# zhouxuguang/GNXRayTracer

Hardware: AMD Instinct MI355X
Metric: Mrays/sec + wall-clock to 1024spp, dragon Cornell 1920×1080 (higher is better)
Workload: dtype f32; 1 GPU; cfg3: Cornell + synthetic 100000-tri mesh (stand-in for absent dragon.3d), Glass+Metal, PathIntegrator maxDepth 8 rr 1 spatial, Halton(1024), 1920x1080; passes_in_flight=4, sub_passes=56, spp_rendered=1024, gather=n/a, world_size=1, backend=none, devices_visible=1

## Files before the change

gnxraytracer_amd/__init__.py:

```python
import collections
import ctypes as C
import os

import numpy as np

from . import _abi
from ._abi import (Camera, Hit, Light, LiSample, Material, Medium, Ray, RenderParams, SceneDesc, Stats, Texture)

_HERE = os.path.dirname(os.path.abspath(__file__))
LIB_PATH = os.environ.get("GNXR_LIB", os.path.join(_HERE, "libgnxr.so"))


class GnxrError(RuntimeError):
    pass


_lib = None
_device = 0


def lib():
    global _lib
    if _lib is None:
        if not os.path.exists(LIB_PATH):
# ... 265 lines not shown
            if d.lights[i].type == _abi.LIGHT_INFINITE:
                self._env_light = Light()
                C.memmove(C.byref(self._env_light), C.byref(d.lights[i]), C.sizeof(Light))
                break
        self._textures = []
        for i in range(int(d.n_textures)):
            t = Texture()
            C.memmove(C.byref(t), C.byref(d.textures[i]), C.sizeof(Texture))
            t.texel_offset = 0
            self._textures.append(t)
        _check(lib().gnxr_scene_create(C.byref(d), C.byref(self._h)))

    def close(self):
        if getattr(self, "_h", None) and _lib is not None:
            _lib.gnxr_scene_destroy(self._h)
            self._h = None

    __del__ = close

    def info(self):
        n, dmax, nv = C.c_int32(), C.c_int32(), C.c_int32()
        _check(lib().gnxr_scene_info(self._h, C.byref(n), C.byref(dmax), C.byref(nv)))
        return {"bvh_nodes": n.value, "bvh_max_depth": dmax.value, "light_voxels": nv.value}

    def update_vertices(self, xyz, first_vertex=0, stream=None, move_lights=False):
        if isinstance(xyz, np.ndarray):
            if xyz.dtype != np.float32 or xyz.ndim != 2 or xyz.shape[1] != 3:
                raise ValueError(f"update_vertices: expected a float32 array of shape (n, 3), got {xyz.dtype} {xyz.shape}")
            xyz = np.ascontiguousarray(xyz)
            ptr = xyz.ctypes.data
        elif type(xyz).__module__.split(".")[0] == "torch":
            import torch
            if not (isinstance(xyz, torch.Tensor) and xyz.is_cuda and xyz.device.index == self.device and xyz.dtype == torch.float32 and
                    xyz.dim() == 2 and xyz.shape[1] == 3 and xyz.is_contiguous()):
                raise ValueError(f"update_vertices: expected a contiguous float32 (n, 3) tensor on cuda:{self.device}, got "
                                 f"{getattr(xyz, 'dtype', None)} {tuple(getattr(xyz, 'shape', ()))} on {getattr(xyz, 'device', None)}")
            ptr = xyz.data_ptr()
            if stream is None:
                stream = torch.cuda.current_stream(xyz.device)
        else:
            raise ValueError(f"update_vertices: expected a numpy array or a torch tensor, got {type(xyz).__name__}")
        stream = _stream_handle("update_vertices", stream)
        if move_lights:
            _check(lib().gnxr_scene_update_vertices_ex(self._h, int(first_vertex), int(xyz.shape[0]), C.c_void_p(ptr or None), _abi.UPDATE_MOVE_LIGHTS,
                                                       C.c_void_p(stream or None)))
        else:
# ... 1041 lines not shown
```

gnxraytracer_amd/_abi.py:

```python
import ctypes as C

GNXR_ABI_VERSION = 5

OK, ERR_INVALID, ERR_NO_DEVICE, ERR_OOM, ERR_UNSUPPORTED, ERR_IO, ERR_RUNTIME = 0, -1, -2, -3, -4, -5, -6
MAT_NONE, MAT_MATTE, MAT_MIRROR, MAT_GLASS, MAT_METAL, MAT_PLASTIC, MAT_DISNEY = range(7)
LIGHT_AREA_TRI, LIGHT_INFINITE, LIGHT_SKYBOX, LIGHT_POINT, LIGHT_SPOT, LIGHT_DISTANT = 1, 2, 3, 4, 5, 6
INTEGRATOR_PATH, INTEGRATOR_VOLPATH, INTEGRATOR_WHITTED, INTEGRATOR_DIRECT = 0, 1, 2, 3
DIRECT_SAMPLE_ALL, DIRECT_SAMPLE_ONE = 0, 1
LIGHTS_SPATIAL, LIGHTS_UNIFORM, LIGHTS_POWER = 0, 1, 2
MEDIUM_HOMOGENEOUS, MEDIUM_GRID = 1, 2
DMEDIUM_BYTES = 128
DLIGHT_BYTES = 112
DTEXTURE_BYTES = 112
UPDATE_MOVE_LIGHTS = 1

f32, i32, u8, i64, u32, u64 = C.c_float, C.c_int32, C.c_uint8, C.c_int64, C.c_uint32, C.c_uint64


class Material(C.Structure):
    _fields_ = [
        ("type", i32), ("has_bump", i32), ("remap_roughness", i32), ("disney_thin", i32),
        ("kd", f32 * 3), ("ks", f32 * 3), ("kr", f32 * 3), ("kt", f32 * 3), ("eta", f32 * 3), ("k", f32 * 3),
        ("sigma", f32), ("urough", f32), ("vrough", f32),
        ("disney_metallic", f32), ("disney_spec_trans", f32), ("disney_spec_tint", f32), ("disney_sheen", f32),
# ... 140 lines not shown
    "gnxr_scene_create": (C.c_int, [P(SceneDesc), P(VP)]),
    "gnxr_scene_destroy": (None, [VP]),
    "gnxr_scene_info": (C.c_int, [VP, P(i32), P(i32), P(i32)]),
    "gnxr_scene_update_vertices": (C.c_int, [VP, i32, i32, VP, VP]),
    "gnxr_scene_update_vertices_ex": (C.c_int, [VP, i32, i32, VP, u32, VP]),
    "gnxr_scene_update_lights": (C.c_int, [VP, i32, i32, P(Light)]),
    "gnxr_scene_set_lights": (C.c_int, [VP, P(Light), i32, VP]),
    "gnxr_scene_light_tables": (C.c_int, [VP, i32, VP, i64, P(i64)]),
    "gnxr_scene_rebuild_bvh": (C.c_int, [VP, VP]),
    "gnxr_scene_set_geometry": (C.c_int, [VP, P(Geometry), VP]),
    "gnxr_scene_update_environment": (C.c_int, [VP, P(Light), VP, i32, i32, VP]),
    "gnxr_scene_env_tables": (C.c_int, [VP, i32, VP, i64, P(i64)]),
    "gnxr_scene_update_media": (C.c_int, [VP, i32, i32, P(Medium), VP, VP]),
    "gnxr_scene_media_tables": (C.c_int, [VP, i32, i32, VP, i64, P(i64)]),
    "gnxr_scene_update_textures": (C.c_int, [VP, i32, i32, P(Texture), VP, VP]),
    "gnxr_scene_texture_tables": (C.c_int, [VP, i32, i32, VP, i64, P(i64)]),
    "gnxr_scene_update_materials": (C.c_int, [VP, i32, i32, P(Material)]),
    "gnxr_scene_set_triangle_materials": (C.c_int, [VP, i32, i32, VP, VP]),
    "gnxr_scene_triangle_materials": (C.c_int, [VP, P(i32), P(C.c_uint8), C.c_int64]),
    "gnxr_scene_set_camera": (C.c_int, [VP, P(Camera), i32]),
    "gnxr_render": (C.c_int, [VP, P(RenderParams), P(f32), P(Stats)]),
    "gnxr_render_device": (C.c_int, [VP, P(RenderParams), VP, VP, P(Stats)]),
    "gnxr_render_reserve": (C.c_int, [VP, P(RenderParams)]),
    "gnxr_trace_closest": (C.c_int, [VP, P(Ray), i64, P(Hit)]),
    "gnxr_trace_any": (C.c_int, [VP, P(Ray), i64, P(u8)]),
    "gnxr_trace_closest_device": (C.c_int, [VP, VP, i64, VP, VP]),
    "gnxr_trace_any_device": (C.c_int, [VP, VP, i64, VP, VP]),
    "gnxr_li_device": (C.c_int, [VP, P(RenderParams), VP, VP, i64, VP, VP, P(Stats)]),
    "gnxr_render_views_device": (C.c_int, [VP, P(RenderParams), P(Camera), P(i32), i32, VP, VP, P(Stats)]),
    "gnxr_render_aov_device": (C.c_int, [VP, P(RenderParams), P(Camera), P(i32), i32, P(AovBuffers), VP, P(Stats)]),
    "gnxr_render_adaptive_device": (C.c_int, [VP, P(RenderParams), P(AdaptiveParams), VP, VP, VP, P(Stats), P(AdaptiveInfo)]),
    "gnxr_denoise_device": (C.c_int, [P(DenoiseParams), P(DenoiseBuffers), VP, VP]),
    "gnxr_film_filter_table": (C.c_int, [P(FilmFilter), P(f32)]),
    "gnxr_film_add_device": (C.c_int, [P(FilmFilter), i32, i32, i32, i32, VP, VP, VP, VP]),
    "gnxr_film_resolve_device": (C.c_int, [i32, i32, i32, VP, VP, VP]),
    "gnxr_render_filtered_device": (C.c_int, [VP, P(RenderParams), P(FilmFilter), P(Camera), P(i32), i32, VP, VP, u32, VP, P(Stats)]),
    "gnxr_material_albedo": (C.c_int, [P(Material), P(f32)]),
    "gnxr_camera_rays_device": (C.c_int, [P(Camera), i32, i32, i32, VP, VP, VP, i64, VP, VP, VP]),
    "gnxr_bsdf_device": (C.c_int, [VP, VP, VP, VP, VP, i64, i32, VP, VP]),
    "gnxr_light_sample_device": (C.c_int, [VP, VP, i64, i32, VP, VP]),
    "gnxr_light_le_device": (C.c_int, [VP, i32, VP, i64, VP, VP]),
    "gnxr_sample_halton": (C.c_int, [i32, i32, P(i32), P(i32), P(i64), P(i32), i64, P(f32)]),
    "gnxr_camera_rays": (C.c_int, [P(Camera), i32, i32, P(i32), P(i32), P(i64), i64, P(f32), P(f32)]),
    "gnxr_framebuffer_update": (C.c_int, [P(f32), P(f32), i32, i32, i32, P(u8)]),
    "gnxr_framebuffer_save_png": (C.c_int, [C.c_char_p, P(u8), i32, i32]),
    "gnxr_light_grid_table": (C.c_int, [VP, i32, i32, P(f32), i64, P(i64)]),
# ... 52 lines not shown
```

gnxraytracer_amd/csrc/api.hip:

```cpp
#include <hip/hip_runtime.h>

#include <chrono>
#include <cstdio>
#include <cstdlib>
#include <memory>
#include <mutex>
#include <string>
#include <thread>
#include <vector>

#include "host_scene.h"
#include "kernels.hip.h"
#include "trace4_kernel.hip.h"
#include "hlbvh_build.hip.h"
#include "refit_kernel.hip.h"
#include "material_kernel.hip.h"
#include "rebuild_kernel.hip.h"
#include "geometry_kernel.hip.h"
#include "lights_kernel.hip.h"
#include "env_build_kernel.hip.h"
#include "media_kernel.hip.h"
#include "texture_build_kernel.hip.h"
#include "li_kernel.hip.h"
#include "views_kernel.hip.h"
// ... 142 lines not shown
    if (rc) return rc;
    gnxr_scene *s = new (std::nothrow) gnxr_scene(g_device);
    if (!s) return GNXR_ERR_OOM;
    if (!compile_scene(desc, &s->cs, device_hlbvh_build)) { delete s; return GNXR_ERR_INVALID; }
    for (size_t i = 1; i < g_devices.size(); ++i) s->replicas.push_back(std::make_unique<gnxr_scene>(g_devices[i], s->host));
    if ((rc = s->each_copy(upload_scene)) != GNXR_OK) { delete s; return rc; }
    const CompiledScene &cs = s->cs;
    if (getenv("GNXR_VERBOSE"))
        fprintf(stderr, "[gnxr] scene: %zu tris, %zu nodes (depth %d), %zu 4-wide nodes (stack %d), wide=%d, %zu device(s)\n", cs.tris.size(), cs.nodes.size(), cs.bvh_max_depth,
                cs.nodes4.size(), cs.stack4_need, (int)s->wide_ok, s->n_copies());
    *out = s;
    return GNXR_OK;
}
void gnxr_scene_destroy(gnxr_scene *s) { delete s; }

int gnxr_scene_info(const gnxr_scene *s, int32_t *n_nodes, int32_t *max_depth, int32_t *n_vox) {
    if (!s) return GNXR_ERR_INVALID;
    if (n_nodes) *n_nodes = (int32_t)s->cs.nodes.size();
    if (max_depth) *max_depth = s->cs.bvh_max_depth;
    if (n_vox) *n_vox = s->grid_strategy >= 0 ? s->grid.nvox[0] * s->grid.nvox[1] * s->grid.nvox[2] : 0;
    return GNXR_OK;
}

int gnxr_render_device(gnxr_scene *s, const gnxr_render_params *pin, void *d_rgba_out, void *hip_stream, gnxr_stats *stats) {
    return render_sharded(s, pin, d_rgba_out, hip_stream, stats);
}

int gnxr_render_reserve(gnxr_scene *s, const gnxr_render_params *pin) {
    if (!s || !pin) { set_error("null argument"); return GNXR_ERR_INVALID; }
    int dummy = 0;
    return render_sharded(s, pin, &dummy, nullptr, nullptr, true);
}

int gnxr_render(gnxr_scene *s, const gnxr_render_params *p, float *rgba_out, gnxr_stats *stats) {
    if (!s || !p || !rgba_out) { set_error("null argument"); return GNXR_ERR_INVALID; }
    if (p->width <= 0 || p->height <= 0) { set_error("invalid image size"); return GNXR_ERR_INVALID; }
    size_t npx = (size_t)p->width * p->height;
    std::lock_guard<std::recursive_mutex> lock(s->render_mutex);
    if (int brc = s->bind()) return brc;
    const bool grew = !(s->out.p && npx <= s->out.n);
    int rc = s->out.alloc(npx);
    if (rc) return rc;
    HIP_TRY(hipMemset(s->out.p, 0, npx * sizeof(float4)));
    rc = render_sharded(s, p, s->out.p, nullptr, stats);
    if (rc) { if (grew) s->out.release(); return rc; }
    int sc = p->shard_count > 0 ? p->shard_count : 1, sr = p->shard_rows > 0 ? p->shard_rows : 1;
// ... 254 lines not shown
```

gnxraytracer_amd/csrc/api_common.hip.h:

```cpp
#pragma once

namespace { int hip_status(hipError_t e); }
#define HIP_TRY(expr)                                                                                   \
    do {                                                                                                \
        hipError_t e_ = (expr);                                                                         \
        if (e_ != hipSuccess) {                                                                         \
            set_error("%s failed: %s (%s:%d)", #expr, hipGetErrorString(e_), __FILE__, __LINE__);       \
            return hip_status(e_);                                                                      \
        }                                                                                               \
    } while (0)

namespace {

int hip_status(hipError_t e) {
    if (e == hipErrorOutOfMemory) return GNXR_ERR_OOM;
    if (e == hipErrorNoDevice || e == hipErrorInvalidDevice || e == hipErrorInsufficientDriver || e == hipErrorNotInitialized) return GNXR_ERR_NO_DEVICE;
    return GNXR_ERR_RUNTIME;
}

int g_device = -1;
std::vector<int> g_devices;
std::vector<char> g_peer_ok;
int g_num_cus = 256;
int g_profiling = 0;
// ... 27 lines not shown
#define GX_ONCE(type, expr) do { static const type v = (expr); return v; } while (0)
    static int trace_blocks_per_cu() { const int v = env_int("GNXR_TRACE_BLOCKS_PER_CU", 0); return v >= 1 && v <= 8 ? v : 0; }
    static int grid_blocks_per_cu() { const int v = env_int("GNXR_GRID_BLOCKS_PER_CU", 0); return v >= 1 && v <= 4096 ? v : 0; }
    static int trace_lds_levels() { GX_ONCE(int, env_set("GNXR_TRACE_LDS_LEVELS") ? std::max(2, env_int("GNXR_TRACE_LDS_LEVELS", 0)) : 64); }
    static int trace_chunk() { GX_ONCE(int, env_set("GNXR_TRACE_CHUNK") ? std::max(64, env_int("GNXR_TRACE_CHUNK", 0) / 64 * 64) : kTraceChunk); }
    static bool leaf_box_table() { GX_ONCE(bool, env_set("GNXR_LEAF_BOX_TABLE")); }
    static int regions() { GX_ONCE(int, env_int("GNXR_REGIONS", 0)); }
    static bool pipeline() { GX_ONCE(bool, env_int("GNXR_PIPELINE", 1) != 0); }
    static int pipe_cut() { GX_ONCE(int, env_int("GNXR_PIPE_CUT", -1)); }
    static int loop_lag() { GX_ONCE(int, env_int("GNXR_LOOP_LAG", -1)); }
    static int shade_blocks_per_cu() { GX_ONCE(int, env_set("GNXR_SHADE_BLOCKS_PER_CU") ? std::max(1, env_int("GNXR_SHADE_BLOCKS_PER_CU", 0)) : 32); }
    static int shade_lds_dims() { GX_ONCE(int, env_set("GNXR_SHADE_LDS_DIMS") ? std::max(0, std::min(128, env_int("GNXR_SHADE_LDS_DIMS", 0))) : 64); }
    static bool shade_lds_tables() { GX_ONCE(bool, env_int("GNXR_SHADE_LDS_TABLES", 1) != 0); }
    static int shade_streams() { GX_ONCE(int, env_int("GNXR_SHADE_STREAMS", -1)); }
    static bool vol_pack() { GX_ONCE(bool, env_int("GNXR_VOL_PACK", 1) != 0); }
#undef GX_ONCE
    static int volmedia_step_cap() { return env_set("GNXR_VOLMEDIA_STEP_CAP") ? std::max(0, env_int("GNXR_VOLMEDIA_STEP_CAP", 0)) : 64; }
    static bool no_escape_queue() { return env_set("GNXR_NO_ESCAPE_QUEUE"); }
    static bool no_material_queues() { return env_set("GNXR_NO_MATERIAL_QUEUES"); }
    static bool no_narrow_shade() { return env_set("GNXR_NO_NARROW_SHADE"); }
    static bool no_mis_defer() { return env_set("GNXR_NO_MIS_DEFER"); }
    static int mis_defer_step() { const int v = env_int("GNXR_MIS_DEFER_STEP", 2); return v == 1 ? 1 : 2; }
    static int mis_defer_drain_at() { return std::max(1, std::min(64, env_int("GNXR_MIS_DEFER_DRAIN_AT", 64))); }
    static bool host_light_grid() { return env_set("GNXR_HOST_LIGHT_GRID"); }
    static bool binary_bvh() { return env_set("GNXR_BINARY_BVH"); }
};

int ensure_device() {
    if (g_device >= 0) { HIP_TRY(hipSetDevice(g_device)); return GNXR_OK; }
    int n = 0;
    hipError_t e = hipGetDeviceCount(&n);
    if (e != hipSuccess || n <= 0) {
        set_error("no HIP device available (%s); libgnxr has no CPU fallback", e != hipSuccess ? hipGetErrorString(e) : "0 devices");
        return GNXR_ERR_NO_DEVICE;
    }
    int dev = 0;
    HIP_TRY(hipGetDevice(&dev));
    hipDeviceProp_t prop;
    HIP_TRY(hipGetDeviceProperties(&prop, dev));
    g_num_cus = prop.multiProcessorCount > 0 ? prop.multiProcessorCount : 256;
    g_device = dev;
    if (const int v = Knobs::trace_blocks_per_cu()) g_trace_blocks_per_cu = v;
    if (const int v = Knobs::grid_blocks_per_cu()) g_grid_bpc = v;
    return GNXR_OK;
}

// ... 32 lines not shown
```

gnxraytracer_amd/csrc/api_render.hip.h:

```cpp
#pragma once

struct TraceLaunch {
    int entries;
    int lds_entries;
    bool spill_needed;
    size_t lds;
    int n_top;
    int blocks;
};
static TraceLaunch trace_launch(const gnxr_scene *s, bool wide, bool spheres, long long total) {
    TraceLaunch t;
    t.entries = wide ? s->cs.stack4_need + 1 : s->cs.bvh_max_depth + 2;
    const int per_cu = g_trace_blocks_per_cu;
    const size_t fixed_b = wide ? (size_t)(kRayRecDwords + (spheres ? 1 : 0)) * kRqStride * sizeof(int) + (size_t)kTopCache * 128 + kOrderTableBytes : 0;
    t.lds_entries = std::min(std::min(t.entries, Knobs::trace_lds_levels()), std::max(2, (int)(((160 * 1024) / per_cu - 1024 - fixed_b) / (kBlock * sizeof(int)))));
    t.spill_needed = t.entries > t.lds_entries;
    t.lds = (size_t)t.lds_entries * kBlock * sizeof(int) + fixed_b;
    t.n_top = (int)std::min<size_t>(kTopCache, s->cs.root4 >= 0 ? s->cs.nodes4.size() : 0);
    t.blocks = (int)std::min<long long>((long long)g_num_cus * per_cu, (total + kBlock - 1) / kBlock);
    return t;
}

static int count_local_rows(const gnxr_render_params *p) {
    int rows = 0;
// ... 526 lines not shown

#define GX_CHECK_LAUNCHES(where)                                                                                    \
    do {                                                                                                            \
        const hipError_t le_ = hipGetLastError();                                                                   \
        if (le_ != hipSuccess) { set_error("HIP runtime error in " where ": %s", hipGetErrorString(le_)); return hip_status(le_); } \
    } while (0)

static int run_path_loop(RenderRun &run) {
    gnxr_scene *s = run.s;
    RenderState &st = run.st;
    const RenderPlan &pl = run.pl;
    hipStream_t stream = run.stream;
    Counters *dctr = run.dctr;
    const size_t half = pl.half;
    struct Sub { long long u0; int kk; };
    std::vector<Sub> subs;
    for (long long u0 = pl.unit_begin; u0 < pl.unit_end; u0 += pl.k) subs.push_back(Sub{u0, (int)std::min<long long>(pl.k, pl.unit_end - u0)});
    const int R = pl.in_flight;
    struct Region { int sub = -1, started = -1; long long paths = 0; } reg[kMaxRegions];
    const int lag = std::max(1, std::min(gnxr_scene::kRing - 2, Knobs::loop_lag() >= 0 ? Knobs::loop_lag() : 2));
    const int stagger = Knobs::pipe_cut() >= 0 ? Knobs::pipe_cut() : std::max(1, (pl.p.max_depth + 2 + lag + R - 1) / R);
    int *qbuf[2] = {st.queue_a.p, st.queue_b.p};
    int in_idx = 0;
    const unsigned *cnt_ptr = &dctr->n_queue;
    size_t next_sub = 0, done_subs = 0;
    int iter = 0, last_start = -(1 << 20), newest_seen = -1;
    int ring_iter[gnxr_scene::kRing];
    for (int &v : ring_iter) v = -1;
    Counters seen;
    memset(&seen, 0, sizeof(seen));
    long long guard = 0;
    while (done_subs < subs.size()) {
        {
            int oldest_needed = iter - 1 - lag;
            for (int j = newest_seen + 1; j <= oldest_needed; ++j) {
                const int slot = j % gnxr_scene::kRing;
                if (j >= 0 && ring_iter[slot] == j) HIP_TRY(hipEventSynchronize(s->ring_ev[slot]));
            }
            for (int j = iter - 1; j > newest_seen; --j) {
                const int slot = ((j % gnxr_scene::kRing) + gnxr_scene::kRing) % gnxr_scene::kRing;
                if (j < 0 || ring_iter[slot] != j) continue;
                const hipError_t q = hipEventQuery(s->ring_ev[slot]);
                if (q == hipSuccess) { seen = s->h_ring[slot]; newest_seen = j; if (int rc = compact_stalled(seen)) return rc; break; }
                if (q != hipErrorNotReady) { set_error("HIP runtime error in the path loop: hipEventQuery: %s", hipGetErrorString(q)); return hip_status(q); }
                (void)hipGetLastError();
            }
// ... 29 lines not shown
            HIP_TRY(hipEventRecord(s->ring_ev[slot], stream));
            ring_iter[slot] = iter;
        }
        int trace_idx = out_idx;
        long long n_trace_upper = n_upper;
        int free_rg = -1;
        for (int rg = 0; rg < R && free_rg < 0; ++rg) if (reg[rg].sub < 0) free_rg = rg;
        const bool start = next_sub < subs.size() && free_rg >= 0 && (!any_active || iter - last_start >= stagger);
        if (start) {
            const Sub &nw = subs[next_sub];
            const int n_new = (int)(pl.unit * nw.kk);
            const size_t base = (size_t)free_rg * half;
            run.raygen(run.pa.at(base), nw.u0, nw.kk, nullptr);
            hipLaunchKernelGGL(k_queue_merge, dim3(grid_for(n_upper + n_new)), dim3(kBlock), 0, stream, (const int *)qbuf[out_idx], dctr, any_active ? 0 : 1, free_rg, (int)base, n_new, qbuf[in_idx]);
            run.launches += 2;
            trace_idx = in_idx; n_trace_upper = n_upper + n_new;
            run.new_paths += (unsigned long long)n_new;
            reg[free_rg].sub = (int)next_sub; reg[free_rg].started = iter; reg[free_rg].paths = n_new;
            last_start = iter;
            ++next_sub;
        }
        if (any_active || start) {
            TraceWork tw{qbuf[trace_idx], (int)n_trace_upper, st.queue_nee.p, any_active ? (int)n_upper : 0, nullptr, reinterpret_cast<unsigned char *>(st.nee_vis.p), cnt_ptr,
                         any_active ? (const unsigned *)&dctr->q_nee : nullptr};
            run.launch_trace(tw, 0, 0, false);
            if (any_active) {
                if (run.timing) run.timer.begin(1, stream);
                hipLaunchKernelGGL(k_nee_combine, dim3(grid_for(n_upper)), dim3(kBlock), 0, stream, run.pa, (const int *)st.queue_nee.p, (int)n_upper, reinterpret_cast<const unsigned char *>(st.nee_vis.p),
                                   (const unsigned *)&dctr->q_nee);
                if (run.timing) run.timer.end(stream);
                ++run.launches;
            }
            in_idx = trace_idx;
        }
        GX_CHECK_LAUNCHES("the path loop");
        ++iter; ++run.loop_iterations;
        if (++guard > (1ll << 24)) { set_error("path loop did not terminate"); return GNXR_ERR_INVALID; }
    }
    return GNXR_OK;
}

static int run_whitted_pass(RenderRun &run, long long u0, int kk) {
    RenderState &st = run.st;
    const RenderPlan &pl = run.pl;
    hipStream_t stream = run.stream;
    Counters *dctr = run.dctr;
    const DScene &sc = run.sc;
    const DRender &r = run.r;
    const PathArrays &pa = run.pa;
    const WhittedArrays &wa = run.wa;
    const int n_paths = (int)(pl.unit * kk), n_records = pl.n_records;
    const bool textured = pl.textured_scene;
// ... 353 lines not shown
```

gnxraytracer_amd/csrc/kernels.hip.h:

```cpp
#pragma once
#include "device_bsdf.h"
#include "device_lights.h"
#include "device_texture.h"

namespace gnxr {

constexpr int kBlock = 256;

constexpr int kRS = 2;
constexpr int kRSm = 2 * kRS;
constexpr int kRecGroups = 5;
struct PathArrays {
    float4 *ray_o;
    float4 *ray_d;
    float4 *beta;
    uint2 *meta;
    float4 *L;
    int *hit;
    unsigned char *pflags;
    unsigned char *pclass;
    float4 *sh_o;
    float4 *sh_d;
    float4 *sh_X;
    float4 *nbeta;
// ... 17 lines not shown
    }
};

constexpr int kMaxRegions = 8;
struct Counters {
    unsigned long long nodes, tris;
    unsigned int q_next, q_nee, q_shadow, q_mis;
    unsigned int q_low;
    unsigned int q_class[4];
    unsigned int cursor;
    unsigned long long whitted_shadow;
    unsigned long long whitted_mis;
    unsigned long long media_steps;
    unsigned long long media_cont;
    unsigned long long retests;
    unsigned long long nodes_global;
    unsigned int n_queue;
    unsigned int iter;
    unsigned int region_lb[kMaxRegions + 1];
    unsigned int region_alive[kMaxRegions];
    unsigned long long rays_continue, rays_shadow, rays_mis;
    unsigned long long li_bad;
    unsigned int compact_stall;
};

struct DScene {
    const float4 *nodes;
    const float4 *nodes4;
    int root4;
    const DTri *tris;
    const unsigned char *tri_class;
    const float4 *leaf_box;
    int leaf1_from_verts;
    const DSphere *spheres;
    int n_spheres;
    int escape_class;
    const DMaterial *materials;
    DLightTables lt;
    DSamplerTables st;
};

struct DRender {
    DCamera cam;
    int W, H, spp, max_depth;
    float rr_threshold;
    int shard_index, shard_count, shard_rows;
// ... 877 lines not shown
```

gnxraytracer_amd/csrc/trace4_kernel.hip.h:

```cpp
#pragma once
#include "kernels.hip.h"
#include "query_kernel.hip.h"
#include "wide_collapse.h"

namespace gnxr {

GX_DEV unsigned order_entry(unsigned code, unsigned hm) {
    const unsigned byte = wide_order_byte(code);
    unsigned e = 0, n = 0;
    for (int i = 0; i < 4; ++i) {
        const unsigned slot = (byte >> (2 * i)) & 3u;
        if ((hm >> slot) & 1u) { e |= slot << (2u * n); ++n; }
    }
    return e;
}
constexpr int kOrderTableBytes = 256;
#ifndef GX_T4_CACHE
#define GX_T4_CACHE 64
#endif
constexpr int kTopCache = GX_T4_CACHE;
constexpr int kRayRecDwords = 11;
#ifndef GX_T4_RQ
#define GX_T4_RQ 64
#endif
constexpr int kRayQueue = GX_T4_RQ;
constexpr int kRqStride = (kBlock / 64) * kRayQueue;
GX_DEV int trace4_lds_dwords_per_thread(bool sph) { return kRayRecDwords + (sph ? 1 : 0); }

#ifndef GX_T4_WAVES
#define GX_T4_WAVES 5
#endif
#if GX_T4_WAVES > 0
#define GX_T4_BOUNDS __launch_bounds__(kBlock, GX_T4_WAVES)
#else
#define GX_T4_BOUNDS __launch_bounds__(kBlock)
#endif
template <bool COUNT, bool SPH, bool SPILL, int Q = kT4Render>
__global__ void GX_T4_BOUNDS k_trace4(DScene sc, typename Trace4Src<Q>::type pa, TraceWork w, unsigned int *cursor, Counters *ctr, int lds_entries, int *spill, int chunk, int n_top) {
    extern __shared__ int smem[];
    typedef __attribute__((address_space(3))) float lds_float;
    lds_int *const stk = (lds_int *)&smem[threadIdx.x];
    global_int *const spl = (global_int *)(spill + (size_t)blockIdx.x * kBlock + threadIdx.x);
    const int spillStride = (int)gridDim.x * kBlock;
    const int lane = __lane_id();
    lds_int *const rq = (lds_int *)&smem[lds_entries * kBlock + (threadIdx.x >> 6) * kRayQueue];
    trace_work_counts(w);
    const unsigned total = (unsigned)w.n_closest + (unsigned)w.n_nee;
    chunk = trace_chunk(total, chunk);
    const ChunkPlan plan = chunk_plan(total, (unsigned)chunk);
// ... 14 lines not shown
    {
        const f4v *gn = reinterpret_cast<const f4v *>(sc.nodes4);
        for (int i = threadIdx.x; i < n_top * 8; i += kBlock) topN[(i & 7) * kTopCache + (i >> 3)] = gn[i];
        if (threadIdx.x < kOrderTableBytes) lut[threadIdx.x] = (unsigned char)order_entry(threadIdx.x >> 4, threadIdx.x & 15u);
        __syncthreads();
    }

    auto push = [&](int &n, int v) {
        if (!SPILL || n < lds_entries) stk[n * kBlock] = v;
        else spl[(n - lds_entries) * spillStride] = v;
        ++n;
    };
    auto pop = [&](int &n) -> int {
        --n;
        return (!SPILL || n < lds_entries) ? stk[n * kBlock] : spl[(n - lds_entries) * spillStride];
    };

#ifndef GX_T4_REFILL_IN_A
#define GX_T4_REFILL_IN_A 0
#endif
    unsigned poolBase = 0, poolCount = 0;
    bool exhausted = false;
    unsigned rqHead = 0, rqCount = 0;

    bool live = false;
    int pk = 0, path = -1;
    constexpr int kMisOwed = 256;
    V3 ro, inv;
    float Sx = 0, Sy = 0, tMax = 0;
    unsigned oNX = 0, oNY = 16, oNZ = 32;
    unsigned ordShift = 0;
    int cur = -1, toVisit = 0, leafOff = 0, leafN = 0, hitLeaf = -1;
    uint32_t cntNodes = 0, cntTris = 0, cntRetests = 0, cntNodesGlobal = 0;
#ifdef GX_TRACE_STATS
    unsigned long long st_[24] = {0};
#endif

    auto take_ray = [&](unsigned slot) {
        const lds_float *q = (const lds_float *)(rq + slot);
        ro = V3(q[0 * kRqStride], q[1 * kRqStride], q[2 * kRqStride]); tMax = q[3 * kRqStride];
        inv = V3(q[4 * kRqStride], q[5 * kRqStride], q[6 * kRqStride]); Sx = q[7 * kRqStride];
        Sy = q[8 * kRqStride];
        pk = (pk & kMisOwed) | __float_as_int(q[9 * kRqStride]);
        path = __float_as_int(q[10 * kRqStride]);
        hitLeaf = SPH ? rq[slot + 11 * kRqStride] : -1;
        const int neg0 = inv.x < 0, neg1 = inv.y < 0, neg2 = inv.z < 0;
        oNX = neg0 ? 48u : 0u; oNY = neg1 ? 64u : 16u; oNZ = neg2 ? 80u : 32u;
        ordShift = 4u * (unsigned)(neg0 | (neg1 << 1) | (neg2 << 2));
        cur = ((pk >> 4) & 1) ? -1 : sc.root4; toVisit = 0; leafN = 0;
        live = true;
    };
    auto retire_ray = [&]() {
        const int kind = pk & 3;
        if constexpr (Q == kT4QueryClosest) pa.hits[path].prim = hitLeaf;
        else if constexpr (Q == kT4QueryAny) pa.occluded[path] = hitLeaf != -1 ? 1 : 0;
        else if (kind == 0) {
            pa.hit[path] = hitLeaf;
            if (hitLeaf < 0) {
                int cls = sc.escape_class;
                if (SPH && hitLeaf != -1) { const int mat = sc.spheres[-2 - hitLeaf].material; if (mat >= 0) cls = sc.materials[mat].shade_class; }
                else if (sc.lt.n_infinite == 0) {
                    cls = 4;
                    pa.pflags[path] = 0;
                }
                pa.pclass[path] = (unsigned char)cls;
            }
        }
        else if (kind == 1) {
            if (w.vis) w.vis[4 * (size_t)path] = hitLeaf == -1 ? 1 : 0;
            else reinterpret_cast<float *>(&pa.sh_o[(size_t)path * kRS])[3] = hitLeaf == -1 ? 1.f : 0.f;
        } else {
            const int expect = __float_as_int(pa.mis_o[(size_t)path * kRS].w);
            bool ok = (expect >= 0) ? (hitLeaf == expect) : (hitLeaf == -1);
            if (w.vis) w.vis[4 * (size_t)path + 1] = ok ? 1 : 0;
            else reinterpret_cast<float *>(&pa.mis_o[(size_t)path * kRS])[3] = ok ? 1.f : 0.f;
        }
        live = false;
    };
#ifdef GX_TRACE_STATS
#define GX_TICK(i) do { const unsigned long long t_ = __builtin_amdgcn_s_memtime(); GX_STAT(i, t_ - tick_); tick_ = t_; } while (0)
    unsigned long long tick_ = __builtin_amdgcn_s_memtime();
#else
#define GX_TICK(i) do {} while (0)
#endif
    while (true) {
        GX_STAT(0, 1);
        GX_TICK(15);
        const bool need = !live;
        const unsigned long long needMask = __ballot(need);
        if (needMask) {
            if (rqCount == 0) {
                const bool misPass = Q == kT4Render && __ballot((pk & kMisOwed) != 0) != 0;
                if (!misPass && poolCount == 0 && !exhausted) {
                    unsigned v = waveId;
                    if (!firstFetch) {
                        if (lane == 0) v = nWaves + atomicAdd(cursor, 1u);
                        v = __shfl(v, 0);
                    }
                    firstFetch = false;
                    if (!chunk_range(plan, v, total, &poolBase, &poolCount)) { exhausted = true; poolCount = 0; }
#ifdef GX_TAIL_STAMP
                    if (Q == kT4Render && !tailSeen && (exhausted || poolBase + poolCount >= tailFrom)) {
                        tailSeen = true;
                        if (lane == 0) atomicMin(&g_tail[0], (unsigned long long)wall_clock64());
                    }
#endif
                }
                if (misPass || poolCount > 0) {
                    const unsigned take = min(poolCount, (unsigned)kRayQueue);
                    bool valid = false, wantMis = false;
                    float4 r0 = make_float4(0, 0, 0, 0), r1 = r0, r2 = r0;
                    int sphHit = -1;
                    if (misPass ? (pk & kMisOwed) != 0 : (unsigned)lane < take) {
                        unsigned i = poolBase + (unsigned)lane;
                        if (w.order) i = w.order[i];
                        float4 o4, d4;
                        int kind_ = 0, path_, any_ = 0;
                        float tMax_;
                        valid = true;
                        if constexpr (Q != kT4Render) {
                            path_ = (int)i;
                            o4 = pa.rays[2 * (size_t)i]; d4 = pa.rays[2 * (size_t)i + 1];
                            tMax_ = o4.w;
                            kind_ = Q == kT4QueryAny ? 1 : 0; any_ = kind_;
                        } else if (i < (unsigned)w.n_closest) {
                            path_ = w.q_closest ? w.q_closest[i] : (int)i;
                            o4 = pa.ray_o[(size_t)path_ * kRS]; d4 = pa.ray_d[(size_t)path_ * kRS];
                            tMax_ = o4.w;
                        } else {
                            path_ = w.q_nee[i - (unsigned)w.n_closest];
                            if (!misPass) {
                                kind_ = 1; any_ = 1;
                                o4 = pa.sh_o[(size_t)path_ * kRS]; d4 = pa.sh_d[(size_t)path_ * kRS]; tMax_ = o4.w;
                                const int nflags = __float_as_int(d4.w);
                                valid = (nflags & 1) != 0;
                                wantMis = (nflags & 2) != 0;
                            } else {
                                kind_ = 2;
                                o4 = pa.mis_o[(size_t)path_ * kRS]; d4 = pa.mis_d[(size_t)path_ * kRS];
                                tMax_ = GX_INF;
                                any_ = __float_as_int(o4.w) < 0 ? 1 : 0;
                            }
                        }
                        if (valid) {
                            const V3 o(o4.x, o4.y, o4.z), d(d4.x, d4.y, d4.z);
                            const V3 iv(1.f / d.x, 1.f / d.y, 1.f / d.z);
                            const RayShear sh = ray_shear(d);
                            int done = 0;
                            for (int si = 0; SPH && si < sc.n_spheres; ++si) {
                                float tH;
                                if (sphere_test(sc.spheres[si], o, d, tMax_, &tH)) {
                                    sphHit = -2 - si;
                                    if (any_) { done = 1; break; }
                                    tMax_ = tH;
                                }
                            }
                            const int ex = (__builtin_isinf(iv.x) || __builtin_isinf(iv.y) || __builtin_isinf(iv.z)) ? 1 : 0;
                            r0 = make_float4(o.x, o.y, o.z, tMax_);
                            r1 = make_float4(iv.x, iv.y, iv.z, sh.Sx);
                            r2 = make_float4(sh.Sy, __int_as_float(kind_ | (sh.kz << 2) | (done << 4) | (ex << 5) | (any_ << 6)), __int_as_float(path_), 0.f);
                        }
                    }
                    const unsigned long long vm = __ballot(valid);
                    if (valid) {
                        const int slot = __popcll(vm & ((1ull << lane) - 1ull));
                        lds_float *q = (lds_float *)(rq + slot);
                        q[0 * kRqStride] = r0.x; q[1 * kRqStride] = r0.y; q[2 * kRqStride] = r0.z; q[3 * kRqStride] = r0.w;
                        q[4 * kRqStride] = r1.x; q[5 * kRqStride] = r1.y; q[6 * kRqStride] = r1.z; q[7 * kRqStride] = r1.w;
                        q[8 * kRqStride] = r2.x; q[9 * kRqStride] = r2.y; q[10 * kRqStride] = r2.z;
                        if (SPH) rq[slot + 11 * kRqStride] = sphHit;
                    }
                    __builtin_amdgcn_fence(__ATOMIC_SEQ_CST, "wavefront");
                    rqCount = (unsigned)__popcll(vm); rqHead = 0;
                    bool advance = true;
                    if (Q == kT4Render) {
                        if (misPass) pk &= ~kMisOwed;
                        else if (wantMis) pk |= kMisOwed;
                        advance = misPass || __ballot(wantMis) == 0;
                    }
                    if (advance) { poolBase += take; poolCount -= take; }
                    GX_STAT(7, 1);
                    GX_STAT(8, misPass ? rqCount : take);
                }
            }
            if (rqCount > 0) {
                const unsigned rank = (unsigned)__popcll(needMask & ((1ull << lane) - 1ull));
                if (need && rank < rqCount) take_ray(rqHead + rank);
                const unsigned t = min(rqCount, (unsigned)__popcll(needMask));
                rqHead += t; rqCount -= t;
                __builtin_amdgcn_fence(__ATOMIC_SEQ_CST, "wavefront");
            }
        }
        GX_TICK(11);
        const unsigned long long liveMask = __ballot(live);
        if (liveMask == 0) {
            if (exhausted && rqCount == 0 && poolCount == 0) break;
// ... 141 lines not shown
                    const float4 b1 = make_float4(fmaxf(fmaxf(p0.y, p1.y), p2.y), fmaxf(fmaxf(p0.z, p1.z), p2.z), 0.f, 0.f);
                    inBox = slab_test(b0, b1, ro, inv, neg, tMax);
                }
                more = leafN > 1;
#ifdef GX_COUNT_TRI_TESTS
                if (COUNT && inBox) cntTris++;
#endif
                TriHit h;
                if (inBox && tri_test_sheared(p0, p1, p2, ro, shear, tMax, &h)) {
                    hitLeaf = leafOff;
                    if (pk & 64) { cur = -1; more = false; }
                    else tMax = h.t;
                }
            }
            if (more) { leafOff += 1; leafN -= 1; pk |= 128; }
            else { leafN = 0; pk &= ~128; }
        }
        GX_TICK(13);
        if (live && cur == -1 && leafN == 0) retire_ray();
    }
#ifdef GX_TRACE_STATS
    if (lane == 0) for (int i = 0; i < 24; ++i) if (st_[i]) atomicAdd(&g_trace_stats[i], st_[i]);
#endif
    if (COUNT) {
        atomicAdd(&ctr->nodes, (unsigned long long)cntNodes);
        atomicAdd(&ctr->tris, (unsigned long long)cntTris);
        atomicAdd(&ctr->retests, (unsigned long long)cntRetests);
        atomicAdd(&ctr->nodes_global, (unsigned long long)cntNodesGlobal);
    }
#ifdef GX_TAIL_STAMP
    if (Q == kT4Render && lane == 0) {
        atomicMax(&g_tail[1], (unsigned long long)wall_clock64());
        __threadfence();
        if (atomicAdd(&g_tail[3], 1ull) == (unsigned long long)nWaves - 1ull) {
            __threadfence();
            const unsigned long long tEnd = atomicExch(&g_tail[1], 0ull), tCross = atomicExch(&g_tail[0], ~0ull), tStart = atomicExch(&g_tail[2], ~0ull);
            atomicExch(&g_tail[3], 0ull);
            const unsigned long long behind = tEnd > tCross ? tEnd - tCross : 0ull, all = tEnd > tStart ? tEnd - tStart : 0ull;
            const int o = total >= (1u << 24) ? 8 : 4;
            g_tail[o] += behind; g_tail[o + 1] += all; g_tail[o + 2] += 1ull; g_tail[o + 3] += total;
            if (o == 8) { g_tail[4] += behind; g_tail[5] += all; g_tail[6] += 1ull; g_tail[7] += total; }
        }
    }
#endif
}

// ... 2 lines not shown
```

gnxraytracer_amd/csrc/trace_kernel.hip.h:

```cpp
#pragma once
#include "device_geom.h"

namespace gnxr {

struct TraceWork {
    const int *q_closest; int n_closest;
    const int *q_nee; int n_nee;
    const unsigned *order;
    unsigned char *vis;
    const unsigned *n_closest_dev, *n_nee_dev;
};
GX_DEV void trace_work_counts(TraceWork &w) {
    if (w.n_closest_dev) { w.n_closest = (int)*w.n_closest_dev; w.n_nee = w.n_nee_dev ? (int)*w.n_nee_dev : 0; }
}
GX_DEV int trace_chunk(unsigned total, int chunk_max) {
    const unsigned waves = gridDim.x * (blockDim.x / 64u);
    const unsigned per = ((total + waves - 1u) / waves + 63u) / 64u * 64u;
    return (int)min((unsigned)chunk_max, max(64u, per));
}

#ifndef GX_CHUNK_TAIL
#define GX_CHUNK_TAIL 384
#endif
#ifndef GX_CHUNK_MID
#define GX_CHUNK_MID 256
#endif
struct ChunkPlan { unsigned c, big, k1, mid_end, k2; };
GX_DEV ChunkPlan chunk_plan(unsigned total, unsigned c) {
    const unsigned waves = gridDim.x * (blockDim.x / 64u);
    ChunkPlan p;
    p.c = c;
    const unsigned tail = waves * (unsigned)GX_CHUNK_TAIL;
    p.big = (c > 128u && total > tail) ? (total - tail) / c * c : 0u;
// ... 315 lines not shown
                }
            }
            else if (kind == 1) {
                if (w.vis) w.vis[4 * (size_t)path] = hitLeaf == -1 ? 1 : 0;
                else reinterpret_cast<float *>(&pa.sh_o[(size_t)path * kRS])[3] = hitLeaf == -1 ? 1.f : 0.f;
            } else {
                bool ok = (expect >= 0) ? (hitLeaf == expect) : (hitLeaf == -1);
                if (w.vis) w.vis[4 * (size_t)path + 1] = ok ? 1 : 0;
                else reinterpret_cast<float *>(&pa.mis_o[(size_t)path * kRS])[3] = ok ? 1.f : 0.f;
            }
            item = -1;
        }
    }
#ifdef GX_TRACE_STATS
    if (lane == 0) for (int i = 0; i < 24; ++i) if (st_[i]) atomicAdd(&g_trace_stats[i], st_[i]);
#endif
    if (COUNT) {
        atomicAdd(&ctr->nodes, (unsigned long long)cntNodes);
        atomicAdd(&ctr->tris, (unsigned long long)cntTris);
        atomicAdd(&ctr->retests, (unsigned long long)cntRetests);
    }
}

static __global__ void __launch_bounds__(kBlock) k_nee_combine(PathArrays pa, const int *__restrict__ queue, int n, const unsigned char *__restrict__ vis, const unsigned *n_dev = nullptr) {
    if (n_dev) n = (int)*n_dev;
    for (int i = blockIdx.x * blockDim.x + threadIdx.x; i < n; i += gridDim.x * blockDim.x) {
        int path = queue[i];
        const unsigned v = reinterpret_cast<const unsigned *>(vis)[path];
        const int flags = (int)((v >> 16) & 0xffu);
        if (!(flags & 0x80) && !(((flags & 1) && (v & 0xffu)) || ((flags & 2) && ((v >> 8) & 0xffu)))) continue;
        float4 X4 = pa.sh_X[(size_t)path * kRS];
        Spec Ld(0.f);
        if ((flags & 1) && (v & 0xffu)) Ld = Ld + Spec(X4.x, X4.y, X4.z);
        if ((flags & 2) && ((v >> 8) & 0xffu)) {
            float4 Y4 = pa.mis_Y[path];
            Spec Y(Y4.x, Y4.y, Y4.z);
            if (!Y.is_black()) Ld = Ld + Y;
        }
        float4 nb = pa.nbeta[(size_t)path * kRS], L4 = pa.L[path];
        Spec add = Spec(nb.x, nb.y, nb.z) * (Ld / X4.w);
        pa.L[path] = make_float4(L4.x + add.r, L4.y + add.g, L4.z + add.b, 0.f);
    }
}

}
```

include/gnxr.h:

```cpp
#ifndef GNXR_H
#define GNXR_H

#include <stdint.h>

#ifdef __cplusplus
extern "C" {
#endif

#define GNXR_ABI_VERSION 5

typedef enum gnxr_status {
    GNXR_OK = 0,
    GNXR_ERR_INVALID = -1,
    GNXR_ERR_NO_DEVICE = -2,
    GNXR_ERR_OOM = -3,
    GNXR_ERR_UNSUPPORTED = -4,
    GNXR_ERR_IO = -5,
    GNXR_ERR_RUNTIME = -6
} gnxr_status;

typedef enum gnxr_material_type {
    GNXR_MAT_NONE = 0,
    GNXR_MAT_MATTE = 1,
    GNXR_MAT_MIRROR = 2,
// ... 262 lines not shown
    const int32_t *tri_medium_inside;
    const int32_t *tri_medium_outside;
    const float   *tri_uv;
    const float   *tri_n;
    const float   *tri_s;
} gnxr_geometry;
int gnxr_scene_set_geometry(gnxr_scene *scene, const gnxr_geometry *g, void *hip_stream);
int gnxr_scene_update_materials(gnxr_scene *scene, int32_t first_material, int32_t n_materials, const gnxr_material *materials);
int gnxr_scene_set_triangle_materials(gnxr_scene *scene, int32_t first_triangle, int32_t n_triangles, const int32_t *material, void *hip_stream);
int gnxr_scene_triangle_materials(gnxr_scene *scene, int32_t *material_out, uint8_t *shade_class_out, int64_t capacity);
int gnxr_scene_env_tables(gnxr_scene *scene, int32_t which, void *out, int64_t capacity_bytes, int64_t *n_bytes);
int gnxr_scene_update_media(gnxr_scene *scene, int32_t first_medium, int32_t n_media, const gnxr_medium *media, const float *density, void *hip_stream);
int gnxr_scene_media_tables(gnxr_scene *scene, int32_t which, int32_t medium, void *out, int64_t capacity_bytes, int64_t *n_bytes);
int gnxr_scene_update_textures(gnxr_scene *scene, int32_t first_texture, int32_t n_textures, const gnxr_texture *textures, const float *texels, void *hip_stream);
int gnxr_scene_texture_tables(gnxr_scene *scene, int32_t which, int32_t texture, void *out, int64_t capacity_bytes, int64_t *n_bytes);
int gnxr_scene_set_camera(gnxr_scene *scene, const gnxr_camera *camera, int32_t camera_medium);

int gnxr_render(gnxr_scene *scene, const gnxr_render_params *params, float *rgba_out,
                gnxr_stats *stats);
int gnxr_render_device(gnxr_scene *scene, const gnxr_render_params *params, void *d_rgba_out,
                       void *hip_stream, gnxr_stats *stats);

int gnxr_render_reserve(gnxr_scene *scene, const gnxr_render_params *params);

int gnxr_trace_closest(gnxr_scene *scene, const gnxr_ray *rays, int64_t n, gnxr_hit *hits);
int gnxr_trace_any(gnxr_scene *scene, const gnxr_ray *rays, int64_t n, uint8_t *occluded);
int gnxr_trace_closest_device(gnxr_scene *scene, const gnxr_ray *d_rays, int64_t n, gnxr_hit *d_hits, void *hip_stream);
int gnxr_trace_any_device(gnxr_scene *scene, const gnxr_ray *d_rays, int64_t n, uint8_t *d_occluded, void *hip_stream);

int gnxr_li_device(gnxr_scene *scene, const gnxr_render_params *params, const gnxr_ray *d_rays, const gnxr_li_sample *d_samples, int64_t n,
                   float *d_L, void *hip_stream, gnxr_stats *stats);

int gnxr_render_views_device(gnxr_scene *scene, const gnxr_render_params *params, const gnxr_camera *cameras, const int32_t *camera_media,
                             int32_t n_views, void *d_rgba_out, void *hip_stream, gnxr_stats *stats);
int gnxr_camera_rays_device(const gnxr_camera *camera, int32_t camera_medium, int32_t width, int32_t height, const int32_t *d_px,
                            const int32_t *d_py, const int32_t *d_s, int64_t n, gnxr_ray *d_rays, gnxr_li_sample *d_samples, void *hip_stream);

typedef struct gnxr_aov_buffers {
    float   *d_albedo;
    float   *d_normal;
    float   *d_shading_normal;
    float   *d_depth;
    int32_t *d_ids;
} gnxr_aov_buffers;
int gnxr_render_aov_device(gnxr_scene *scene, const gnxr_render_params *params, const gnxr_camera *cameras, const int32_t *camera_media,
                           int32_t n_views, const gnxr_aov_buffers *out, void *hip_stream, gnxr_stats *stats);
// ... 97 lines not shown
```

Before: 5359 Mrays/s.

## Apply NEE shadow results inside the trace kernel with a lagged in-wave sweep

The persistent trace kernel now folds completed next-event-estimation shadow/MIS visibility results into path radiance itself, working kNeeLag items behind the batch it is setting up. Each result is marked applied through a per-path flag byte, so the later k_nee_combine sweep skips it. Visibility encoding changes to 2/3 so readiness can be detected. The aim is to cut the global memory traffic and work of the separate combine pass. In exchange it adds extra loads, fences and atomics inside the hot traversal loop, plus counters and an API to report how many results were applied where.

```diff
diff --git a/gnxraytracer_amd/__init__.py b/gnxraytracer_amd/__init__.py
--- a/gnxraytracer_amd/__init__.py
+++ b/gnxraytracer_amd/__init__.py
@@ -311,6 +311,11 @@
         n, dmax, nv = C.c_int32(), C.c_int32(), C.c_int32()
         _check(lib().gnxr_scene_info(self._h, C.byref(n), C.byref(dmax), C.byref(nv)))
         return {"bvh_nodes": n.value, "bvh_max_depth": dmax.value, "light_voxels": nv.value}
+
+    def nee_apply_counts(self):
+        t, w = C.c_uint64(), C.c_uint64()
+        _check(lib().gnxr_scene_nee_apply_counts(self._h, C.byref(t), C.byref(w)))
+        return int(t.value), int(w.value)
 
     def update_vertices(self, xyz, first_vertex=0, stream=None, move_lights=False):
         if isinstance(xyz, np.ndarray):
diff --git a/gnxraytracer_amd/_abi.py b/gnxraytracer_amd/_abi.py
--- a/gnxraytracer_amd/_abi.py
+++ b/gnxraytracer_amd/_abi.py
@@ -186,6 +186,7 @@
     "gnxr_render": (C.c_int, [VP, P(RenderParams), P(f32), P(Stats)]),
     "gnxr_render_device": (C.c_int, [VP, P(RenderParams), VP, VP, P(Stats)]),
     "gnxr_render_reserve": (C.c_int, [VP, P(RenderParams)]),
+    "gnxr_scene_nee_apply_counts": (C.c_int, [VP, P(u64), P(u64)]),
     "gnxr_trace_closest": (C.c_int, [VP, P(Ray), i64, P(Hit)]),
     "gnxr_trace_any": (C.c_int, [VP, P(Ray), i64, P(u8)]),
     "gnxr_trace_closest_device": (C.c_int, [VP, VP, i64, VP, VP]),
diff --git a/gnxraytracer_amd/csrc/api.hip b/gnxraytracer_amd/csrc/api.hip
--- a/gnxraytracer_amd/csrc/api.hip
+++ b/gnxraytracer_amd/csrc/api.hip
@@ -188,6 +188,19 @@
     return GNXR_OK;
 }
 
+int gnxr_scene_nee_apply_counts(gnxr_scene *s, uint64_t *in_trace, uint64_t *by_sweep) {
+    if (!s) { set_error("null argument"); return GNXR_ERR_INVALID; }
+    std::lock_guard<std::recursive_mutex> lock(s->render_mutex);
+    uint64_t t = 0, w = 0;
+    for (size_t i = 0; i <= s->replicas.size(); ++i) {
+        const Counters *c = s->copy(i)->h_counters;
+        if (c) { t += c->nee_applied_trace; w += c->nee_applied_sweep; }
+    }
+    if (in_trace) *in_trace = t;
+    if (by_sweep) *by_sweep = w;
+    return GNXR_OK;
+}
+
 int gnxr_render_device(gnxr_scene *s, const gnxr_render_params *pin, void *d_rgba_out, void *hip_stream, gnxr_stats *stats) {
     return render_sharded(s, pin, d_rgba_out, hip_stream, stats);
 }
diff --git a/gnxraytracer_amd/csrc/api_common.hip.h b/gnxraytracer_amd/csrc/api_common.hip.h
--- a/gnxraytracer_amd/csrc/api_common.hip.h
+++ b/gnxraytracer_amd/csrc/api_common.hip.h
@@ -73,6 +73,7 @@
     static bool no_mis_defer() { return env_set("GNXR_NO_MIS_DEFER"); }
     static int mis_defer_step() { const int v = env_int("GNXR_MIS_DEFER_STEP", 2); return v == 1 ? 1 : 2; }
     static int mis_defer_drain_at() { return std::max(1, std::min(64, env_int("GNXR_MIS_DEFER_DRAIN_AT", 64))); }
+    static bool no_trace_nee_apply() { return env_set("GNXR_NO_TRACE_NEE_APPLY"); }
     static bool host_light_grid() { return env_set("GNXR_HOST_LIGHT_GRID"); }
     static bool binary_bvh() { return env_set("GNXR_BINARY_BVH"); }
 };
diff --git a/gnxraytracer_amd/csrc/api_render.hip.h b/gnxraytracer_amd/csrc/api_render.hip.h
--- a/gnxraytracer_amd/csrc/api_render.hip.h
+++ b/gnxraytracer_amd/csrc/api_render.hip.h
@@ -572,6 +572,7 @@
     const int stagger = Knobs::pipe_cut() >= 0 ? Knobs::pipe_cut() : std::max(1, (pl.p.max_depth + 2 + lag + R - 1) / R);
     int *qbuf[2] = {st.queue_a.p, st.queue_b.p};
     int in_idx = 0;
+    const int nee_in_trace = Knobs::no_trace_nee_apply() ? 0 : 1;
     const unsigned *cnt_ptr = &dctr->n_queue;
     size_t next_sub = 0, done_subs = 0;
     int iter = 0, last_start = -(1 << 20), newest_seen = -1;
@@ -647,12 +648,12 @@
         }
         if (any_active || start) {
             TraceWork tw{qbuf[trace_idx], (int)n_trace_upper, st.queue_nee.p, any_active ? (int)n_upper : 0, nullptr, reinterpret_cast<unsigned char *>(st.nee_vis.p), cnt_ptr,
-                         any_active ? (const unsigned *)&dctr->q_nee : nullptr};
+                         any_active ? (const unsigned *)&dctr->q_nee : nullptr, nee_in_trace};
             run.launch_trace(tw, 0, 0, false);
             if (any_active) {
                 if (run.timing) run.timer.begin(1, stream);
                 hipLaunchKernelGGL(k_nee_combine, dim3(grid_for(n_upper)), dim3(kBlock), 0, stream, run.pa, (const int *)st.queue_nee.p, (int)n_upper, reinterpret_cast<const unsigned char *>(st.nee_vis.p),
-                                   (const unsigned *)&dctr->q_nee);
+                                   (const unsigned *)&dctr->q_nee, &dctr->nee_applied_sweep);
                 if (run.timing) run.timer.end(stream);
                 ++run.launches;
             }
diff --git a/gnxraytracer_amd/csrc/kernels.hip.h b/gnxraytracer_amd/csrc/kernels.hip.h
--- a/gnxraytracer_amd/csrc/kernels.hip.h
+++ b/gnxraytracer_amd/csrc/kernels.hip.h
@@ -63,6 +63,7 @@
     unsigned long long rays_continue, rays_shadow, rays_mis;
     unsigned long long li_bad;
     unsigned int compact_stall;
+    unsigned long long nee_applied_trace, nee_applied_sweep;
 };
 
 struct DScene {
diff --git a/gnxraytracer_amd/csrc/trace4_kernel.hip.h b/gnxraytracer_amd/csrc/trace4_kernel.hip.h
--- a/gnxraytracer_amd/csrc/trace4_kernel.hip.h
+++ b/gnxraytracer_amd/csrc/trace4_kernel.hip.h
@@ -25,6 +25,17 @@
 #endif
 constexpr int kRayQueue = GX_T4_RQ;
 constexpr int kRqStride = (kBlock / 64) * kRayQueue;
+#ifndef GX_T4_NEE_LAG
+#define GX_T4_NEE_LAG 128
+#endif
+constexpr int kNeeLag = GX_T4_NEE_LAG;
+#ifndef GX_T4_NEE_TAIL
+#define GX_T4_NEE_TAIL 0
+#endif
+#ifndef GX_T4_NEE_BESIDE
+#define GX_T4_NEE_BESIDE 0
+#endif
+static_assert(kNeeLag >= 64 && kNeeLag % 64 == 0, "the lagging items must lie behind the batch that is being set up");
 GX_DEV int trace4_lds_dwords_per_thread(bool sph) { return kRayRecDwords + (sph ? 1 : 0); }
 
 #ifndef GX_T4_WAVES
@@ -85,6 +96,7 @@
     unsigned poolBase = 0, poolCount = 0;
     bool exhausted = false;
     unsigned rqHead = 0, rqCount = 0;
+    unsigned nNeeApplied = 0;
 
     bool live = false;
     int pk = 0, path = -1;
@@ -130,15 +142,33 @@
             }
         }
         else if (kind == 1) {
-            if (w.vis) w.vis[4 * (size_t)path] = hitLeaf == -1 ? 1 : 0;
+            if (w.vis) w.vis[4 * (size_t)path] = hitLeaf == -1 ? 3 : 2;
             else reinterpret_cast<float *>(&pa.sh_o[(size_t)path * kRS])[3] = hitLeaf == -1 ? 1.f : 0.f;
         } else {
             const int expect = __float_as_int(pa.mis_o[(size_t)path * kRS].w);
             bool ok = (expect >= 0) ? (hitLeaf == expect) : (hitLeaf == -1);
-            if (w.vis) w.vis[4 * (size_t)path + 1] = ok ? 1 : 0;
+            if (w.vis) w.vis[4 * (size_t)path + 1] = ok ? 3 : 2;
             else reinterpret_cast<float *>(&pa.mis_o[(size_t)path * kRS])[3] = ok ? 1.f : 0.f;
         }
         live = false;
+    };
+    auto nee_round = [&](unsigned first, unsigned lo, unsigned hi) {
+        if constexpr (Q == kT4Render) {
+            __builtin_amdgcn_fence(__ATOMIC_SEQ_CST, "workgroup");
+            const unsigned j = first + (unsigned)lane;
+            bool did = false;
+            if (j >= lo && j < hi) {
+                const int p = w.q_nee[j - (unsigned)w.n_closest];
+                unsigned *vw = reinterpret_cast<unsigned *>(w.vis) + p;
+                const unsigned v = __hip_atomic_load(vw, __ATOMIC_RELAXED, __HIP_MEMORY_SCOPE_WAVEFRONT);
+                if (nee_ready(v)) {
+                    nee_apply(pa, p, v);
+                    reinterpret_cast<unsigned char *>(vw)[3] = 1;
+                    did = true;
+                }
+            }
+            nNeeApplied += (unsigned)__popcll(__ballot(did));
+        }
     };
 #ifdef GX_TRACE_STATS
 #define GX_TICK(i) do { const unsigned long long t_ = __builtin_amdgcn_s_memtime(); GX_STAT(i, t_ - tick_); tick_ = t_; } while (0)
@@ -155,6 +185,14 @@
             if (rqCount == 0) {
                 const bool misPass = Q == kT4Render && __ballot((pk & kMisOwed) != 0) != 0;
                 if (!misPass && poolCount == 0 && !exhausted) {
+#if GX_T4_NEE_TAIL
+                    if (Q == kT4Render && !firstFetch && w.nee_in_trace && w.vis && !w.order && poolBase > (unsigned)w.n_closest) {
+                        const unsigned len = poolBase <= plan.big ? plan.c : (poolBase <= plan.mid_end ? 128u : (poolBase - 1u - plan.mid_end) % 64u + 1u);
+                        const unsigned lo = max(poolBase - len, (unsigned)w.n_closest);
+                        for (unsigned back = (unsigned)kNeeLag; back >= 64u; back -= 64u)
+                            if (poolBase - lo + 64u > back) nee_round(poolBase - back, lo, poolBase);
+                    }
+#endif
                     unsigned v = waveId;
                     if (!firstFetch) {
                         if (lane == 0) v = nWaves + atomicAdd(cursor, 1u);
@@ -171,15 +209,24 @@
                 }
                 if (misPass || poolCount > 0) {
                     const unsigned take = min(poolCount, (unsigned)kRayQueue);
+                    int neeP = -1;
+                    bool neeOn = false;
+                    if constexpr (Q == kT4Render) {
+                        const unsigned chunkEnd = poolBase + poolCount;
+                        const unsigned chunkLen = chunkEnd <= plan.big ? plan.c : (chunkEnd <= plan.mid_end ? 128u : 0u);
+                        const unsigned lo = max(chunkEnd - chunkLen, (unsigned)w.n_closest) + (unsigned)kNeeLag;
+                        neeOn = !misPass && w.nee_in_trace && w.vis && !w.order && poolBase + 63u >= lo;
+                        if (neeOn && poolBase + (unsigned)lane >= lo) neeP = w.q_nee[poolBase + (unsigned)lane - (unsigned)kNeeLag - (unsigned)w.n_closest];
+                    }
                     bool valid = false, wantMis = false;
                     float4 r0 = make_float4(0, 0, 0, 0), r1 = r0, r2 = r0;
                     int sphHit = -1;
+                    float4 o4 = make_float4(0, 0, 0, 0), d4 = o4;
+                    int kind_ = 0, path_ = 0, any_ = 0;
+                    float tMax_ = 0.f;
                     if (misPass ? (pk & kMisOwed) != 0 : (unsigned)lane < take) {
                         unsigned i = poolBase + (unsigned)lane;
                         if (w.order) i = w.order[i];
-                        float4 o4, d4;
-                        int kind_ = 0, path_, any_ = 0;
-                        float tMax_;
                         valid = true;
                         if constexpr (Q != kT4Render) {
                             path_ = (int)i;
@@ -205,6 +252,23 @@
                                 any_ = __float_as_int(o4.w) < 0 ? 1 : 0;
                             }
                         }
+                    }
+                    unsigned neeV = 0;
+#if GX_T4_NEE_BESIDE
+                    float4 neeX = make_float4(0, 0, 0, 0), neeB = neeX, neeL = neeX;
+#endif
+                    if constexpr (Q == kT4Render) {
+                        if (neeOn) {
+                            __builtin_amdgcn_fence(__ATOMIC_SEQ_CST, "workgroup");
+                            if (neeP >= 0) {
+                                neeV = __hip_atomic_load(reinterpret_cast<unsigned *>(w.vis) + neeP, __ATOMIC_RELAXED, __HIP_MEMORY_SCOPE_WAVEFRONT);
+#if GX_T4_NEE_BESIDE
+                                neeX = pa.sh_X[(size_t)neeP * kRS]; neeB = pa.nbeta[(size_t)neeP * kRS]; neeL = pa.L[neeP];
+#endif
+                            }
+                        }
+                    }
+                    {
                         if (valid) {
                             const V3 o(o4.x, o4.y, o4.z), d(d4.x, d4.y, d4.z);
                             const V3 iv(1.f / d.x, 1.f / d.y, 1.f / d.z);
@@ -235,6 +299,20 @@
                     }
                     __builtin_amdgcn_fence(__ATOMIC_SEQ_CST, "wavefront");
                     rqCount = (unsigned)__popcll(vm); rqHead = 0;
+                    if constexpr (Q == kT4Render) {
+                        if (neeOn) {
+                            const bool did = neeP >= 0 && nee_ready(neeV);
+                            if (did) {
+#if GX_T4_NEE_BESIDE
+                                if (nee_adds(neeV)) pa.L[neeP] = nee_sum(pa, neeP, neeV, neeX, neeB, neeL);
+#else
+                                nee_apply(pa, neeP, neeV);
+#endif
+                                reinterpret_cast<unsigned char *>(w.vis)[4 * (size_t)neeP + 3] = 1;
+                            }
+                            nNeeApplied += (unsigned)__popcll(__ballot(did));
+                        }
+                    }
                     bool advance = true;
                     if (Q == kT4Render) {
                         if (misPass) pk &= ~kMisOwed;
@@ -422,6 +500,7 @@
 #ifdef GX_TRACE_STATS
     if (lane == 0) for (int i = 0; i < 24; ++i) if (st_[i]) atomicAdd(&g_trace_stats[i], st_[i]);
 #endif
+    if (Q == kT4Render && nNeeApplied != 0 && lane == 0) atomicAdd(&ctr->nee_applied_trace, (unsigned long long)nNeeApplied);
     if (COUNT) {
         atomicAdd(&ctr->nodes, (unsigned long long)cntNodes);
         atomicAdd(&ctr->tris, (unsigned long long)cntTris);
diff --git a/gnxraytracer_amd/csrc/trace_kernel.hip.h b/gnxraytracer_amd/csrc/trace_kernel.hip.h
--- a/gnxraytracer_amd/csrc/trace_kernel.hip.h
+++ b/gnxraytracer_amd/csrc/trace_kernel.hip.h
@@ -9,6 +9,7 @@
     const unsigned *order;
     unsigned char *vis;
     const unsigned *n_closest_dev, *n_nee_dev;
+    int nee_in_trace;
 };
 GX_DEV void trace_work_counts(TraceWork &w) {
     if (w.n_closest_dev) { w.n_closest = (int)*w.n_closest_dev; w.n_nee = w.n_nee_dev ? (int)*w.n_nee_dev : 0; }
@@ -370,25 +371,47 @@
     }
 }
 
-static __global__ void __launch_bounds__(kBlock) k_nee_combine(PathArrays pa, const int *__restrict__ queue, int n, const unsigned char *__restrict__ vis, const unsigned *n_dev = nullptr) {
+GX_DEV bool nee_adds(unsigned v) {
+    const unsigned flags = (v >> 16) & 0xffu;
+    return (flags & 0x80u) || ((flags & 1u) && (v & 1u)) || ((flags & 2u) && ((v >> 8) & 1u));
+}
+GX_DEV float4 nee_sum(const PathArrays &pa, int path, unsigned v, const float4 &X4, const float4 &nb, const float4 &L4) {
+    const int flags = (int)((v >> 16) & 0xffu);
+    Spec Ld(0.f);
+    if ((flags & 1) && (v & 1u)) Ld = Ld + Spec(X4.x, X4.y, X4.z);
+    if ((flags & 2) && ((v >> 8) & 1u)) {
+        float4 Y4 = pa.mis_Y[path];
+        Spec Y(Y4.x, Y4.y, Y4.z);
+        if (!Y.is_black()) Ld = Ld + Y;
+    }
+    Spec add = Spec(nb.x, nb.y, nb.z) * (Ld / X4.w);
+    return make_float4(L4.x + add.r, L4.y + add.g, L4.z + add.b, 0.f);
+}
+GX_DEV void nee_apply(const PathArrays &pa, int path, unsigned v) {
+    if (!nee_adds(v)) return;
+    const float4 X4 = pa.sh_X[(size_t)path * kRS], nb = pa.nbeta[(size_t)path * kRS], L4 = pa.L[path];
+    pa.L[path] = nee_sum(pa, path, v, X4, nb, L4);
+}
+GX_DEV bool nee_ready(unsigned v) {
+    const unsigned flags = v >> 16;
+    return (!(flags & 1u) || (v & 2u)) && (!(flags & 2u) || (v & 0x200u)) && (v >> 24) == 0;
+}
+
+static __global__ void __launch_bounds__(kBlock) k_nee_combine(PathArrays pa, const int *__restrict__ queue, int n, const unsigned char *__restrict__ vis, const unsigned *n_dev = nullptr,
+                                                               unsigned long long *n_applied = nullptr) {
     if (n_dev) n = (int)*n_dev;
+    unsigned mine = 0;
     for (int i = blockIdx.x * blockDim.x + threadIdx.x; i < n; i += gridDim.x * blockDim.x) {
         int path = queue[i];
         const unsigned v = reinterpret_cast<const unsigned *>(vis)[path];
-        const int flags = (int)((v >> 16) & 0xffu);
-        if (!(flags & 0x80) && !(((flags & 1) && (v & 0xffu)) || ((flags & 2) && ((v >> 8) & 0xffu)))) continue;
-        float4 X4 = pa.sh_X[(size_t)path * kRS];
-        Spec Ld(0.f);
-        if ((flags & 1) && (v & 0xffu)) Ld = Ld + Spec(X4.x, X4.y, X4.z);
-        if ((flags & 2) && ((v >> 8) & 0xffu)) {
-            float4 Y4 = pa.mis_Y[path];
-            Spec Y(Y4.x, Y4.y, Y4.z);
-            if (!Y.is_black()) Ld = Ld + Y;
-        }
-        float4 nb = pa.nbeta[(size_t)path * kRS], L4 = pa.L[path];
-        Spec add = Spec(nb.x, nb.y, nb.z) * (Ld / X4.w);
-        pa.L[path] = make_float4(L4.x + add.r, L4.y + add.g, L4.z + add.b, 0.f);
-    }
-}
-
-}
+        if (v >> 24) continue;
+        nee_apply(pa, path, v);
+        ++mine;
+    }
+    if (n_applied) {
+        for (int o = 32; o > 0; o >>= 1) mine += __shfl_xor(mine, o);
+        if (__lane_id() == 0 && mine) atomicAdd(n_applied, (unsigned long long)mine);
+    }
+}
+
+}
diff --git a/include/gnxr.h b/include/gnxr.h
--- a/include/gnxr.h
+++ b/include/gnxr.h
@@ -308,6 +308,8 @@
                        void *hip_stream, gnxr_stats *stats);
 
 int gnxr_render_reserve(gnxr_scene *scene, const gnxr_render_params *params);
+
+int gnxr_scene_nee_apply_counts(gnxr_scene *scene, uint64_t *in_trace, uint64_t *by_sweep);
 
 int gnxr_trace_closest(gnxr_scene *scene, const gnxr_ray *rays, int64_t n, gnxr_hit *hits);
 int gnxr_trace_any(gnxr_scene *scene, const gnxr_ray *rays, int64_t n, uint8_t *occluded);
```

After: 5424 Mrays/s (median of 6 runs). 1.2% higher.
